# apache/tez

Measured on AMD Instinct MI355X. Metric: shuffled+sorted KV bytes/sec, higher is better.
Workload: dtype u8; 1 GPU; C2: 1e8 rec x (16B unique key + 64B val), 64 partitions, BytesWritable/TezBytesComparator, ordered shuffle; records=100000000, key_bytes=16, partitions=64, parallelism=single

## Files before the change

### tez_amd/csrc/tezsort.hip

```cpp
#include <hip/hip_runtime.h>
#include <cstdint>
#include <cstdio>
#include <cstdlib>
#include <cstring>
#include <string>
#include <vector>
#include <mutex>
#include <algorithm>
#include <sys/stat.h>
#include <sys/types.h>

#include "tezsort.h"

#define WAVE 64
#define BLOCK 256
#define WPB (BLOCK / WAVE)
#define RADIX 256
#define TILE_ROUNDS 12
#define TILE (TILE_ROUNDS * BLOCK)

static thread_local char g_err[1024];
extern "C" const char* tzs_last_error(void) { return g_err; }

#define FAIL(code, ...)                                        \
  do {                                                         \
    snprintf(g_err, sizeof(g_err), __VA_ARGS__);               \
    return (code);                                             \
  } while (0)

#define HIP_CHECK(x)                                                        \
  do {                                                                      \
    hipError_t _e = (x);                                                    \
    if (_e != hipSuccess)                                                   \
      FAIL(-70, "%s:%d HIP error %d (%s) in %s", __FILE__, __LINE__, (int)_e, \
           hipGetErrorString(_e), #x);                                      \
  } while (0)

static uint32_t h_crc_table[256];
static bool h_crc_init_done = false;
static void h_crc_init() {
  if (h_crc_init_done) return;
  for (uint32_t n = 0; n < 256; n++) {
    uint32_t c = n;
    for (int k = 0; k < 8; k++) c = (c & 1) ? (0xEDB88320u ^ (c >> 1)) : (c >> 1);
    h_crc_table[n] = c;
  }
  h_crc_init_done = true;
}
static uint32_t h_crc32(uint32_t crc, const uint8_t* p, size_t n) {
  h_crc_init();
  crc ^= 0xFFFFFFFFu;
  for (size_t i = 0; i < n; i++) crc = h_crc_table[(crc ^ p[i]) & 0xFF] ^ (crc >> 8);
  return crc ^ 0xFFFFFFFFu;
}

static uint32_t gf2_times(const uint32_t* m, uint32_t v) {
  uint32_t s = 0;
  for (int i = 0; v; i++, v >>= 1)
    if (v & 1) s ^= m[i];
  return s;
}
static void gf2_square(uint32_t* sq, const uint32_t* m) {
  for (int i = 0; i < 32; i++) sq[i] = gf2_times(m, m[i]);
}
#define CRC_MATS 40
static uint32_t h_crc_shift_mat[CRC_MATS][32];
static bool h_mats_done = false;
static void h_build_crc_mats() {
  if (h_mats_done) return;
  uint32_t odd[32], even[32];
  odd[0] = 0xEDB88320u;
  for (int i = 1; i < 32; i++) odd[i] = 1u << (i - 1);
  gf2_square(even, odd);
  gf2_square(odd, even);
  gf2_square(even, odd);
  memcpy(h_crc_shift_mat[0], even, sizeof(even));
  for (int k = 1; k < CRC_MATS; k++)
    gf2_square(h_crc_shift_mat[k], h_crc_shift_mat[k - 1]);
  h_mats_done = true;
}
static uint32_t h_crc_shift(uint32_t crc, uint64_t nbytes) {
  h_build_crc_mats();
  for (int k = 0; nbytes; k++, nbytes >>= 1)
    if (nbytes & 1) crc = gf2_times(h_crc_shift_mat[k], crc);
  return crc;
}
static uint32_t h_crc_combine(uint32_t c1, uint32_t c2, uint64_t len2) {
  return h_crc_shift(c1, len2) ^ c2;
}
extern "C" uint32_t tzs_test_crc_combine(uint32_t c1, uint32_t c2, uint64_t len2) {
  return h_crc_combine(c1, c2, len2);
}
extern "C" uint32_t tzs_test_crc32(uint32_t c, const void* p, uint64_t n) {
  return h_crc32(c, (const uint8_t*)p, n);
}

static int h_vint_size(int64_t i) {
  if (i >= -112 && i <= 127) return 1;
  if (i < 0) i = ~i;
  int n = 0;
  while (i != 0) { i = (int64_t)((uint64_t)i >> 8); n++; }
  return n + 1;
}

__device__ __forceinline__ int d_vint_size(int64_t i) {
  if (i >= -112 && i <= 127) return 1;
  uint64_t u = (i < 0) ? ~(uint64_t)i : (uint64_t)i;
  int n = 0;
  while (u != 0) { u >>= 8; n++; }
  return n + 1;
}
__device__ __forceinline__ int d_vint_write(uint8_t* b, int64_t i) {
  if (i >= -112 && i <= 127) { b[0] = (uint8_t)i; return 1; }
  int len = -112;
  if (i < 0) { i = ~i; len = -120; }
  int64_t tmp = i;
  while (tmp != 0) { tmp = (int64_t)((uint64_t)tmp >> 8); len--; }
  b[0] = (uint8_t)len;
  int n = (len < -120) ? -(len + 120) : -(len + 112);
  for (int idx = n; idx != 0; idx--)
    b[n - idx + 1] = (uint8_t)((uint64_t)i >> ((idx - 1) * 8));
  return n + 1;
}
__device__ __forceinline__ int d_vint_decoded_size(int8_t first) {
  if (first >= -112) return 1;
  if (first < -120) return -119 - first;
  return -111 - first;
}

__device__ __forceinline__ int32_t d_hash_bytes(const uint8_t* p, int32_t n) {
  if (n == 16) {
    uint64_t w0, w1;
    __builtin_memcpy(&w0, p, 8);
    __builtin_memcpy(&w1, p + 8, 8);
    int32_t A = 1, B = 0;
#pragma unroll
    for (int j = 0; j < 8; j++) {
      A = (int32_t)((uint32_t)A * 31u) + (int8_t)(uint8_t)(w0 >> (8 * j));
      B = (int32_t)((uint32_t)B * 31u) + (int8_t)(uint8_t)(w1 >> (8 * j));
    }
    uint32_t p8 = 1;
#pragma unroll
    for (int j = 0; j < 8; j++) p8 *= 31u;
    return (int32_t)((uint32_t)A * p8 + (uint32_t)B);
  }
  int32_t h = 1;
  int32_t i = 0;
  for (; i + 8 <= n; i += 8) {
    uint64_t w;
    __builtin_memcpy(&w, p + i, 8);
    for (int j = 0; j < 8; j++)
      h = (int32_t)((uint32_t)h * 31u) + (int8_t)(uint8_t)(w >> (8 * j));
  }
  for (; i < n; i++) h = (int32_t)((uint32_t)h * 31u) + (int8_t)p[i];
  return h;
}

struct SegDesc {
  const uint8_t* data;
  const uint64_t* off;
  const uint32_t* klen;
  uint32_t rec_u;
  uint32_t klen_u;
};
struct RecTable {
  const uint8_t* data0;
  const uint64_t* off0;
  const uint32_t* klen0;
  const SegDesc* segs;
  const uint32_t* base;
  uint32_t rec_u0, klen_u0;
  uint32_t n0;
  int32_t nspills;
  int32_t key_type;
};

__device__ __forceinline__ int rt_spill_of(const RecTable& rt, uint32_t g) {
  if (rt.nspills == 1 || g < rt.n0) return 0;
  uint32_t lo = 1, hi = (uint32_t)rt.nspills;
  while (lo + 1 < hi) {
    uint32_t mid = (lo + hi) >> 1;
    if (rt.base[mid] <= g) lo = mid; else hi = mid;
  }
  return (int)lo;
}
struct RecView {
  const uint8_t* key;
  uint32_t klen;
  const uint8_t* val;
  uint32_t vlen;
  const uint8_t* content;
  uint32_t clen;
};
__device__ __forceinline__ RecView rt_view(const RecTable& rt, uint32_t g) {
  const uint8_t* data;
  const uint64_t* off;
  const uint32_t* klen;
  uint32_t rec_u, klen_u, r;
  if (rt.nspills == 1 || g < rt.n0) {
    data = rt.data0; off = rt.off0; klen = rt.klen0;
    rec_u = rt.rec_u0; klen_u = rt.klen_u0; r = g;
  } else {
    int s = rt_spill_of(rt, g);
    SegDesc sd = rt.segs[s];
    data = sd.data; off = sd.off; klen = sd.klen;
    rec_u = sd.rec_u; klen_u = sd.klen_u; r = g - rt.base[s];
  }
  RecView v;
  if (rec_u) {
    v.key = data + (uint64_t)r * rec_u;
    v.klen = klen_u;
    v.val = v.key + v.klen;
    v.vlen = rec_u - v.klen;
  } else {
    uint64_t o = off[r];
    v.key = data + o;
    v.klen = klen[r];
    v.val = v.key + v.klen;
    v.vlen = (uint32_t)(off[r + 1] - o - v.klen);
  }
  if (rt.key_type == 1) {
    int n = d_vint_decoded_size((int8_t)v.key[0]);
    v.content = v.key + n;
    v.clen = v.klen - n;
  } else {
    v.content = v.key + 4;
    v.clen = v.klen - 4;
  }
  return v;
}

__global__ void k_shift_offsets(const uint64_t* src, uint64_t* dst, uint64_t shift,
                                int64_t n);
__global__ void k_max_u32(const uint32_t* a, uint32_t n, uint32_t* out);
__global__ void k_part_hist(const uint32_t* parts, uint32_t n, uint32_t* counts, int P);
__global__ void k_gather_part_meta(const uint64_t* pstart, const uint64_t* scan,
                                   const uint8_t* same, uint64_t total_body,
                                   uint32_t n, int P, uint64_t* out);
__global__ void k_check_uniform(const uint64_t* off, const uint32_t* klen, int64_t n,
                                uint64_t* mm );

__global__ void k_hash_partition(RecTable rt, int32_t P, int32_t* d_part, uint32_t n) {
  uint32_t stride = gridDim.x * blockDim.x;
  for (uint32_t i = blockIdx.x * blockDim.x + threadIdx.x; i < n; i += 2 * stride) {
    uint32_t j = i + stride;
    RecView v0 = rt_view(rt, i);
    int32_t h0 = d_hash_bytes(v0.content, (int32_t)v0.clen);
    if (j < n) {
      RecView v1 = rt_view(rt, j);
      int32_t h1 = d_hash_bytes(v1.content, (int32_t)v1.clen);
      d_part[j] = (h1 & 0x7fffffff) % P;
    }
    d_part[i] = (h0 & 0x7fffffff) % P;
  }
}

__device__ __forceinline__ uint64_t d_composite_one(
    const RecTable& rt, const int32_t* d_part, int32_t P, int pbits,
    int ref_pb, int ser_mode, uint64_t mask, uint32_t i) {
  RecView v = rt_view(rt, i);
  uint32_t part;
  if (d_part) part = (uint32_t)d_part[i];
  else part = (uint32_t)((d_hash_bytes(v.content, (int32_t)v.clen) & 0x7fffffff) % P);
  uint64_t key;
  if (ser_mode) {
    uint32_t proxy = ((v.clen > 0 ? (uint32_t)v.content[0] : 0u) << 16) |
                     ((v.clen > 1 ? (uint32_t)v.content[1] : 0u) << 8) |
                     (v.clen > 2 ? (uint32_t)v.content[2] : 0u);
    int pw = 24 - ref_pb;
    if (pw < 0) pw = 0;
    uint32_t proxy_t = pw ? (proxy >> (24 - pw)) : 0;
    uint64_t ser = 0;
    uint32_t m = v.klen < 8 ? v.klen : 8;
    for (uint32_t b = 0; b < m; b++) ser |= (uint64_t)v.key[b] << (56 - 8 * b);
    key = ((uint64_t)part << (64 - pbits))
          | ((uint64_t)proxy_t << (64 - pbits - pw))
          | (ser >> (pbits + pw));
  } else {
    uint64_t c = 0;
    uint32_t m = v.clen < 8 ? v.clen : 8;
    for (uint32_t b = 0; b < m; b++) c |= (uint64_t)v.content[b] << (56 - 8 * b);
    key = pbits ? (((uint64_t)part << (64 - pbits)) | (c >> pbits)) : c;
  }
  return key & mask;
}

__global__ void k_build_composite2(RecTable rt, const int32_t* d_part, int32_t P,
                                   int pbits, int ref_pb, int sort_bytes,
                                   int ser_mode, uint64_t* d_key, uint32_t* d_idx,
                                   uint32_t n) {
  uint64_t mask = (sort_bytes >= 8) ? ~0ull : ~0ull << (8 * (8 - sort_bytes));
  uint32_t stride = gridDim.x * blockDim.x;
  for (uint32_t i = blockIdx.x * blockDim.x + threadIdx.x; i < n; i += 4 * stride) {
    uint32_t i1 = i + stride, i2 = i + 2 * stride, i3 = i + 3 * stride;
    uint64_t k0 = d_composite_one(rt, d_part, P, pbits, ref_pb, ser_mode, mask, i);
    uint64_t k1 = (i1 < n) ? d_composite_one(rt, d_part, P, pbits, ref_pb,
                                             ser_mode, mask, i1) : 0;
    uint64_t k2 = (i2 < n) ? d_composite_one(rt, d_part, P, pbits, ref_pb,
                                             ser_mode, mask, i2) : 0;
    uint64_t k3 = (i3 < n) ? d_composite_one(rt, d_part, P, pbits, ref_pb,
                                             ser_mode, mask, i3) : 0;
    d_key[i] = k0;
    d_idx[i] = i;
    if (i1 < n) { d_key[i1] = k1; d_idx[i1] = i1; }
    if (i2 < n) { d_key[i2] = k2; d_idx[i2] = i2; }
    if (i3 < n) { d_key[i3] = k3; d_idx[i3] = i3; }
  }
}

__global__ void k_build_composite(RecTable rt, const int32_t* d_part, int32_t P,
                                  int pbits, int ref_pb, int sort_bytes, int ser_mode,
                                  uint64_t* d_key, uint32_t* d_idx, uint32_t n) {
  uint64_t mask = (sort_bytes >= 8) ? ~0ull : ~0ull << (8 * (8 - sort_bytes));
  for (uint32_t i = blockIdx.x * blockDim.x + threadIdx.x; i < n;
       i += gridDim.x * blockDim.x) {
    RecView v = rt_view(rt, i);
    uint32_t part;
    if (d_part) part = (uint32_t)d_part[i];
    else part = (uint32_t)((d_hash_bytes(v.content, (int32_t)v.clen) & 0x7fffffff) % P);
    uint64_t key;
    if (ser_mode) {
      uint32_t proxy = ((v.clen > 0 ? (uint32_t)v.content[0] : 0u) << 16) |
                       ((v.clen > 1 ? (uint32_t)v.content[1] : 0u) << 8) |
                       (v.clen > 2 ? (uint32_t)v.content[2] : 0u);
      int pw = 24 - ref_pb;
      if (pw < 0) pw = 0;
      uint32_t proxy_t = pw ? (proxy >> (24 - pw)) : 0;
      uint64_t ser = 0;
      uint32_t m = v.klen < 8 ? v.klen : 8;
      for (uint32_t b = 0; b < m; b++) ser |= (uint64_t)v.key[b] << (56 - 8 * b);
      key = ((uint64_t)part << (64 - pbits))
            | ((uint64_t)proxy_t << (64 - pbits - pw))
            | (ser >> (pbits + pw));
    } else {
      uint64_t c = 0;
      uint32_t m = v.clen < 8 ? v.clen : 8;
      for (uint32_t b = 0; b < m; b++) c |= (uint64_t)v.content[b] << (56 - 8 * b);
      key = pbits ? (((uint64_t)part << (64 - pbits)) | (c >> pbits)) : c;
    }
    d_key[i] = key & mask;
    d_idx[i] = i;
  }
}

template <typename KeyT, int BLK = BLOCK>
__global__ void k_radix_hist(const KeyT* keys, uint32_t n, int byte_idx,
                             uint32_t* counts ) {
  constexpr uint32_t OT = (uint32_t)TILE_ROUNDS * BLK;
  __shared__ uint32_t h[RADIX];
  for (int i = threadIdx.x; i < RADIX; i += blockDim.x) h[i] = 0;
  __syncthreads();
  uint32_t start = blockIdx.x * OT;
  uint32_t end = min(start + OT, n);
  for (uint32_t i = start + threadIdx.x; i < end; i += blockDim.x) {
    uint32_t d = (uint32_t)(keys[i] >> (8 * byte_idx)) & 0xFF;
    atomicAdd(&h[d], 1u);
  }
  __syncthreads();
  for (int i = threadIdx.x; i < RADIX; i += blockDim.x)
    counts[blockIdx.x * RADIX + i] = h[i];
}

__global__ void k_radix_scan_blocks(const uint32_t* counts, uint32_t nblocks,
                                    uint32_t* offsets, uint32_t* totals) {
  int d = blockIdx.x;
  __shared__ uint32_t lds[BLOCK];
  uint32_t running = 0;
  for (uint32_t b0 = 0; b0 < nblocks; b0 += blockDim.x) {
    uint32_t b = b0 + threadIdx.x;
    uint32_t v = (b < nblocks) ? counts[b * RADIX + d] : 0;
    lds[threadIdx.x] = v;
    __syncthreads();
    for (int s = 1; s < BLOCK; s <<= 1) {
      uint32_t t = (threadIdx.x >= (uint32_t)s) ? lds[threadIdx.x - s] : 0;
      __syncthreads();
      lds[threadIdx.x] += t;
      __syncthreads();
    }
    if (b < nblocks) offsets[b * RADIX + d] = running + lds[threadIdx.x] - v;
    uint32_t chunk_total = lds[BLOCK - 1];
    running += chunk_total;
    __syncthreads();
  }
  if (threadIdx.x == 0) totals[d] = running;
}

__global__ void k_radix_scan_digits(uint32_t* totals, uint32_t* bases) {
  __shared__ uint32_t lds[RADIX];
  int t = threadIdx.x;
  lds[t] = totals[t];
  __syncthreads();
  for (int s = 1; s < RADIX; s <<= 1) {
    uint32_t v = (t >= s) ? lds[t - s] : 0;
    __syncthreads();
    lds[t] += v;
    __syncthreads();
  }
  bases[t] = lds[t] - totals[t];
}

template <typename KeyT, bool HAS_A1, bool HAS_B64 = false, int BLK = BLOCK>
__global__ __launch_bounds__(BLK) void k_radix_scatter(
    const KeyT* keys_in, KeyT* keys_out,
    const uint32_t* a0_in, uint32_t* a0_out,
    const uint32_t* a1_in, uint32_t* a1_out,
    const uint64_t* b64_in, uint64_t* b64_out,
    uint32_t n, int byte_idx,
    const uint32_t* offsets, const uint32_t* bases) {
  constexpr uint32_t OT = (uint32_t)TILE_ROUNDS * BLK;
  constexpr int OWPB = BLK / WAVE;
  constexpr int RW = OWPB * TILE_ROUNDS;
  constexpr size_t CNT_BYTES = (size_t)RW * RADIX * 2;
  constexpr size_t KEY_BYTES = (size_t)OT * sizeof(KeyT);
  constexpr size_t UNION_BYTES = CNT_BYTES > KEY_BYTES ? CNT_BYTES : KEY_BYTES;
  __shared__ __attribute__((aligned(16))) uint8_t u_raw[UNION_BYTES];
  __shared__ uint32_t ls_a0[OT];
  __shared__ uint32_t ls_a1[HAS_A1 ? OT : 1];
  __shared__ uint64_t ls_b64[HAS_B64 ? OT : 1];
  __shared__ uint32_t tileoff[RADIX];
  uint16_t* cnt = (uint16_t*)u_raw;
  KeyT* ls_key = (KeyT*)u_raw;
  for (uint32_t i = threadIdx.x; i < (uint32_t)RW * RADIX / 2; i += blockDim.x)
    ((uint32_t*)cnt)[i] = 0;
  __syncthreads();
  uint32_t start = blockIdx.x * OT;
  uint32_t end = min(start + OT, n);
  uint32_t count = (start < n) ? (end - start) : 0;
  const int lane = threadIdx.x & (WAVE - 1);
  const int wv = threadIdx.x / WAVE;
  const uint64_t lt_mask = (lane == 0) ? 0ull : (~0ull >> (64 - lane));
  KeyT my_key[TILE_ROUNDS];
  uint32_t my_a0[TILE_ROUNDS];
  uint32_t my_a1v[HAS_A1 ? TILE_ROUNDS : 1];
  uint64_t my_b64[HAS_B64 ? TILE_ROUNDS : 1];
  uint16_t my_rank[TILE_ROUNDS];
  uint16_t my_dig[TILE_ROUNDS];
  #pragma unroll
  for (int r = 0; r < TILE_ROUNDS; r++) {
    uint32_t i = start + (uint32_t)r * BLK + threadIdx.x;
    bool active = i < end;
    my_key[r] = active ? keys_in[i] : (KeyT)0;
    my_a0[r] = active ? a0_in[i] : 0;
    if (HAS_A1) my_a1v[r] = active ? a1_in[i] : 0;
    if (HAS_B64) my_b64[r] = active ? b64_in[i] : 0;
  }
  for (int r = 0; r < TILE_ROUNDS; r++) {
    uint32_t i = start + (uint32_t)r * BLK + threadIdx.x;
    bool active = i < end;
    uint32_t d = active ? ((uint32_t)(my_key[r] >> (8 * byte_idx)) & 0xFF) : 0u;
    uint64_t m = ~0ull;
    for (int b = 0; b < 8; b++) {
      uint64_t bb = __ballot((d >> b) & 1);
      m &= ((d >> b) & 1) ? bb : ~bb;
    }
    uint64_t act = __ballot(active);
    m &= act;
    uint32_t lane_rank = (uint32_t)__popcll(m & lt_mask);
    if (active && lane_rank == 0)
      cnt[(r * OWPB + wv) * RADIX + d] = (uint16_t)__popcll(m);
    my_rank[r] = (uint16_t)lane_rank;
    my_dig[r] = (uint16_t)d;
  }
  __syncthreads();
  if (threadIdx.x < RADIX) {
    uint32_t d = threadIdx.x;
    uint32_t running = 0;
    for (int rw = 0; rw < RW; rw++) {
      uint32_t t = cnt[rw * RADIX + d];
      cnt[rw * RADIX + d] = (uint16_t)running;
      running += t;
    }
    tileoff[d] = running;
  }
  __syncthreads();
  if (wv == 0) {
    uint32_t v0 = tileoff[4 * lane], v1 = tileoff[4 * lane + 1],
             v2 = tileoff[4 * lane + 2], v3 = tileoff[4 * lane + 3];
    uint32_t sum = v0 + v1 + v2 + v3;
    uint32_t inc = sum;
    for (int s2 = 1; s2 < WAVE; s2 <<= 1) {
      uint32_t t = __shfl_up(inc, s2);
      if (lane >= s2) inc += t;
    }
    uint32_t base0 = inc - sum;
    tileoff[4 * lane] = base0;
    tileoff[4 * lane + 1] = base0 + v0;
    tileoff[4 * lane + 2] = base0 + v0 + v1;
    tileoff[4 * lane + 3] = base0 + v0 + v1 + v2;
  }
  __syncthreads();
  uint16_t my_slot[TILE_ROUNDS];
  for (int r = 0; r < TILE_ROUNDS; r++) {
    uint32_t d = my_dig[r];
    my_slot[r] = (uint16_t)(tileoff[d] + cnt[(r * OWPB + wv) * RADIX + d] +
                            my_rank[r]);
  }
  __syncthreads();
  for (int r = 0; r < TILE_ROUNDS; r++) {
    uint32_t i = start + (uint32_t)r * BLK + threadIdx.x;
    if (i < end) {
      uint32_t slot = my_slot[r];
      ls_key[slot] = my_key[r];
      ls_a0[slot] = my_a0[r];
      if (HAS_A1) ls_a1[slot] = my_a1v[r];
      if (HAS_B64) ls_b64[slot] = my_b64[r];
    }
  }
  __syncthreads();
  for (uint32_t j = threadIdx.x; j < count; j += blockDim.x) {
    KeyT k = ls_key[j];
    uint32_t d = (uint32_t)(k >> (8 * byte_idx)) & 0xFF;
    uint32_t pos = offsets[blockIdx.x * RADIX + d] + bases[d] + (j - tileoff[d]);
    keys_out[pos] = k;
    a0_out[pos] = ls_a0[j];
    if (HAS_A1) a1_out[pos] = ls_a1[j];
    if (HAS_B64) b64_out[pos] = ls_b64[j];
  }
}

#define OS_AGG (1u << 30)
#define OS_INC (2u << 30)
#define OS_CNT_MASK ((1u << 30) - 1)
typedef unsigned int __attribute__((address_space(1))) os_gu32;

template <typename KeyT>
__global__ void k_global_hist_all(const KeyT* keys, uint32_t n, int first_byte,
                                  int npasses, uint32_t* counts ) {
  extern __shared__ uint32_t lh[];
  for (int i = threadIdx.x; i < npasses * RADIX; i += blockDim.x) lh[i] = 0;
  __syncthreads();
  for (uint32_t i = blockIdx.x * blockDim.x + threadIdx.x; i < n;
       i += gridDim.x * blockDim.x) {
    KeyT k = keys[i];
    for (int p = 0; p < npasses; p++)
      atomicAdd(&lh[p * RADIX + ((uint32_t)(k >> (8 * (first_byte + p))) & 0xFF)], 1u);
  }
  __syncthreads();
  for (int i = threadIdx.x; i < npasses * RADIX; i += blockDim.x)
    if (lh[i]) atomicAdd(&counts[i], lh[i]);
}

__global__ void k_os_bases(const uint32_t* counts, uint32_t* bases) {
  __shared__ uint32_t tot[RADIX];
  int p = blockIdx.x;
  int d = threadIdx.x;
  tot[d] = counts[p * RADIX + d];
  __syncthreads();
  if (d == 0) {
    uint32_t run = 0;
    for (int i = 0; i < RADIX; i++) {
      uint32_t t = tot[i];
      tot[i] = run;
      run += t;
    }
  }
  __syncthreads();
  bases[p * RADIX + d] = tot[d];
}

template <typename KeyT, bool HAS_A1, bool HAS_B64 = false, int BLK = BLOCK>
__global__ __launch_bounds__(BLK) void k_onesweep_pass(
    const KeyT* keys_in, KeyT* keys_out,
    const uint32_t* a0_in, uint32_t* a0_out,
    const uint32_t* a1_in, uint32_t* a1_out,
    const uint64_t* b64_in, uint64_t* b64_out,
    uint32_t n, int byte_idx,
    const uint32_t* bases ,
    uint32_t* status , uint32_t* ticket, uint32_t* error) {
  constexpr uint32_t OT = (uint32_t)TILE_ROUNDS * BLK;
  constexpr int OWPB = BLK / WAVE;
  constexpr int RW = OWPB * TILE_ROUNDS;
  constexpr size_t CNT_BYTES = (size_t)RW * RADIX * 2;
  constexpr size_t KEY_BYTES = (size_t)OT * sizeof(KeyT);
  constexpr size_t UNION_BYTES = CNT_BYTES > KEY_BYTES ? CNT_BYTES : KEY_BYTES;
  __shared__ __attribute__((aligned(16))) uint8_t u_raw[UNION_BYTES];
  __shared__ uint32_t ls_a0[OT];
  __shared__ uint32_t ls_a1[HAS_A1 ? OT : 1];
  __shared__ uint64_t ls_b64[HAS_B64 ? OT : 1];
  __shared__ uint32_t tileoff[RADIX];
  __shared__ uint32_t excl[RADIX];
  __shared__ uint32_t s_tile;
  uint16_t* cnt = (uint16_t*)u_raw;
  KeyT* ls_key = (KeyT*)u_raw;
  if (threadIdx.x == 0) s_tile = atomicAdd(ticket, 1u);
  for (uint32_t i = threadIdx.x; i < (uint32_t)RW * RADIX / 2; i += blockDim.x)
    ((uint32_t*)cnt)[i] = 0;
  __syncthreads();
  const uint32_t tile = s_tile;
  const uint32_t start = tile * OT;
  const uint32_t end = min(start + OT, n);
  const uint32_t count = (start < n) ? (end - start) : 0;
  const int lane = threadIdx.x & (WAVE - 1);
  const int wv = threadIdx.x / WAVE;
  const uint64_t lt_mask = (lane == 0) ? 0ull : (~0ull >> (64 - lane));
  KeyT my_key[TILE_ROUNDS];
  uint32_t my_a0[TILE_ROUNDS];
  uint32_t my_a1v[HAS_A1 ? TILE_ROUNDS : 1];
  uint64_t my_b64[HAS_B64 ? TILE_ROUNDS : 1];
  uint16_t my_rank[TILE_ROUNDS];
  uint16_t my_dig[TILE_ROUNDS];
  #pragma unroll
  for (int r = 0; r < TILE_ROUNDS; r++) {
    uint32_t i = start + (uint32_t)r * BLK + threadIdx.x;
    bool active = i < end;
    my_key[r] = active ? keys_in[i] : (KeyT)0;
    my_a0[r] = active ? a0_in[i] : 0;
    if (HAS_A1) my_a1v[r] = active ? a1_in[i] : 0;
    if (HAS_B64) my_b64[r] = active ? b64_in[i] : 0;
  }
// ... 2230 lines not shown
  uint32_t cur_rec_u = 0;
  uint32_t cur_klen_u = 0;
  bool cur_first_batch = true;
  bool have_explicit_parts = false;
  bool combined_parts_valid = false;
  DBuf combine_data, combine_off, combine_klen;
  uint32_t combine_n = 0;
  bool combine_applied = false;
  std::vector<uint8_t> host_data;
  std::vector<uint64_t> host_off;
  std::vector<uint32_t> host_klen;
  std::vector<int32_t> host_part;
  std::vector<SpillData*> spills;
  DBuf final_ifile;
  int64_t final_len = 0;
  std::vector<tzs_index_record> final_index;
  bool flushed = false;
  tzs_counters ctr = {};
  tzs_times times = {};
  DBuf skey, sidx, eq, same, sizes, scan, parts_sorted;
  DBuf skey_lo;
  DBuf comp_ifile;
  int64_t comp_len = 0;
  std::vector<tzs_index_record> comp_index;
  std::vector<uint64_t> final_rec_ranges;
  HostRT final_hrt;
  RecTable final_rt = {};
  uint32_t final_n = 0;
  DBuf col_data, col_off, col_klen;
};

extern "C" void tzs_conf_default(tzs_conf* c, int32_t num_partitions) {
  memset(c, 0, sizeof(*c));
  c->num_partitions = num_partitions;
  c->key_type = TZS_KEY_BYTES;
  c->value_type = TZS_KEY_BYTES;
  c->comparator = TZS_CMP_TEZBYTES;
  c->rle = -1;
  c->send_empty_partition_details = 1;
  c->io_sort_factor = 100;
  c->final_merge_enabled = 1;
  c->sort_buffer_bytes = 100ll << 20;
  c->device = -1;
  c->world_size = 1;
  c->rank = 0;
  c->combiner = 0;
  c->min_spills_for_combine = 3;
  c->discard_spill_streams = 0;
}

extern "C" int tzs_sorter_create(const tzs_conf* conf, tzs_sorter** out) {
  if (!conf || conf->num_partitions <= 0) FAIL(-22, "bad conf");
  if (ensure_device_constants()) return -70;
  tzs_sorter* s = new tzs_sorter();
  s->conf = *conf;
  s->pbits = pbits_for(conf->num_partitions);
  *out = s;
  return 0;
}

extern "C" int tzs_sorter_write(tzs_sorter* s, const void* key, int32_t klen,
                                const void* val, int32_t vlen, int32_t partition) {
  if (s->host_off.empty()) s->host_off.push_back(0);
  const uint8_t* k = (const uint8_t*)key;
  const uint8_t* v = (const uint8_t*)val;
  s->host_data.insert(s->host_data.end(), k, k + klen);
  s->host_data.insert(s->host_data.end(), v, v + vlen);
  s->host_off.push_back(s->host_data.size());
  s->host_klen.push_back((uint32_t)klen);
  s->host_part.push_back(partition);
  if ((int64_t)s->host_data.size() + 16ll * (int64_t)s->host_klen.size()
      > s->conf.sort_buffer_bytes)
    return tzs_sorter_spill(s);
  return 0;
}

static int absorb_host_staging(tzs_sorter* s) {
  if (s->host_klen.empty()) return 0;
  int64_t n = (int64_t)s->host_klen.size();
  static_assert(sizeof(uint64_t) == 8, "");
  DBuf dd, doff, dkl, dpart;
  if (dd.alloc(s->host_data.size() ? s->host_data.size() : 1)) return -12;
  if (doff.alloc(sizeof(uint64_t) * (n + 1))) return -12;
  if (dkl.alloc(sizeof(uint32_t) * n)) return -12;
  if (dpart.alloc(sizeof(int32_t) * n)) return -12;
  HIP_CHECK(hipMemcpy(dd.p, s->host_data.data(), s->host_data.size(), hipMemcpyHostToDevice));
  HIP_CHECK(hipMemcpy(doff.p, s->host_off.data(), sizeof(uint64_t) * (n + 1), hipMemcpyHostToDevice));
  HIP_CHECK(hipMemcpy(dkl.p, s->host_klen.data(), sizeof(uint32_t) * n, hipMemcpyHostToDevice));
  bool have_parts = true;
  for (auto p : s->host_part) if (p < 0) { have_parts = false; break; }
  HIP_CHECK(hipMemcpy(dpart.p, s->host_part.data(), sizeof(int32_t) * n, hipMemcpyHostToDevice));
  int rc = tzs_sorter_write_batch_device(s, dd.p, (const uint64_t*)doff.p,
                                         (const uint32_t*)dkl.p,
                                         have_parts ? (const int32_t*)dpart.p : nullptr, n);
  dd.release(); doff.release(); dkl.release(); dpart.release();
  s->host_data.clear(); s->host_off.clear(); s->host_klen.clear(); s->host_part.clear();
  return rc;
}

#include <chrono>
extern "C" int tzs_sorter_write_batch_device(tzs_sorter* s, const void* d_data,
                                             const uint64_t* d_off, const uint32_t* d_klen,
                                             const int32_t* d_part, int64_t n) {
  auto t0 = std::chrono::steady_clock::now();
  if (n == 0) return 0;
  if (n > 4000000000ll) FAIL(-22, "batch too large (u32 record ids)");
  uint64_t nbytes = 0, first = 0;
  HIP_CHECK(hipMemcpy(&first, d_off, 8, hipMemcpyDeviceToHost));
  HIP_CHECK(hipMemcpy(&nbytes, d_off + n, 8, hipMemcpyDeviceToHost));
  nbytes -= first;
  if (first != 0) FAIL(-22, "d_off must start at 0");

  uint64_t old_bytes = s->cur_bytes;
  int64_t old_n = s->cur_n;
  DBuf nd, noff, nkl, npart;
  if (nd.alloc(old_bytes + nbytes ? old_bytes + nbytes : 1)) return -12;
  if (noff.alloc(sizeof(uint64_t) * (old_n + n + 1))) return -12;
  if (nkl.alloc(sizeof(uint32_t) * (old_n + n))) return -12;
  if (npart.alloc(sizeof(int32_t) * (old_n + n))) return -12;
  if (old_n) {
    HIP_CHECK(hipMemcpyAsync(nd.p, s->cur_data.p, old_bytes, hipMemcpyDeviceToDevice));
    HIP_CHECK(hipMemcpyAsync(noff.p, s->cur_off.p, sizeof(uint64_t) * old_n, hipMemcpyDeviceToDevice));
    HIP_CHECK(hipMemcpyAsync(nkl.p, s->cur_klen.p, sizeof(uint32_t) * old_n, hipMemcpyDeviceToDevice));
    HIP_CHECK(hipMemcpyAsync(npart.p, s->cur_part.p, sizeof(int32_t) * old_n, hipMemcpyDeviceToDevice));
  }
  HIP_CHECK(hipMemcpyAsync((uint8_t*)nd.p + old_bytes, d_data, nbytes, hipMemcpyDeviceToDevice));
  HIP_CHECK(hipMemcpyAsync((uint32_t*)nkl.p + old_n, d_klen, sizeof(uint32_t) * n, hipMemcpyDeviceToDevice));
  hipLaunchKernelGGL(k_shift_offsets, dim3(grid1d(n + 1)), dim3(BLOCK), 0, 0,
                     d_off, (uint64_t*)noff.p + old_n, old_bytes, n + 1);
  std::swap(s->cur_data, nd); nd.release();
  std::swap(s->cur_off, noff); noff.release();
  std::swap(s->cur_klen, nkl); nkl.release();
  if (d_part) {
    HIP_CHECK(hipMemcpyAsync((int32_t*)npart.p + old_n, d_part, sizeof(int32_t) * n,
                             hipMemcpyDeviceToDevice));
    s->have_explicit_parts = true;
  } else if (s->have_explicit_parts) {
    FAIL(-22, "cannot mix explicit and computed partitions in one sorter");
  }
  std::swap(s->cur_part, npart); npart.release();
  {
    static thread_local DBuf mm;
    if (mm.alloc(32)) return -12;
    uint64_t init[4] = {~0ull, 0, ~0ull, 0};
    HIP_CHECK(hipMemcpyAsync(mm.p, init, 32, hipMemcpyHostToDevice));
    hipLaunchKernelGGL(k_check_uniform, dim3(grid1d(n)), dim3(BLOCK), 0, 0,
                       d_off, d_klen, n, (uint64_t*)mm.p);
    uint64_t res[4];
    HIP_CHECK(hipMemcpy(res, mm.p, 32, hipMemcpyDeviceToHost));
    bool uni = (res[0] == res[1]) && (res[2] == res[3]) && res[0] <= 0xFFFFFFFFull;
    if (getenv("TZS_NO_UNIFORM")) uni = false;
    if (s->cur_first_batch) {
      s->cur_rec_u = uni ? (uint32_t)res[0] : 0;
      s->cur_klen_u = uni ? (uint32_t)res[2] : 0;
      s->cur_first_batch = false;
    } else if (!uni || s->cur_rec_u != (uint32_t)res[0] ||
               s->cur_klen_u != (uint32_t)res[2]) {
      s->cur_rec_u = 0;
      s->cur_klen_u = 0;
    }
  }
  s->cur_n = old_n + n;
  s->cur_bytes = old_bytes + nbytes;
  s->ctr.output_records += n;
  s->ctr.output_bytes += (int64_t)nbytes;
  HIP_CHECK(hipDeviceSynchronize());
  s->times.absorb_ns += std::chrono::duration_cast<std::chrono::nanoseconds>(
      std::chrono::steady_clock::now() - t0).count();
  return 0;
}

extern "C" int tzs_sorter_write_batch_device_adopt(tzs_sorter* s, void* d_data,
                                                   uint64_t* d_off, uint32_t* d_klen,
                                                   int32_t* d_part, int64_t n) {
  auto t0 = std::chrono::steady_clock::now();
  if (n == 0) return 0;
  if (n > 4000000000ll) FAIL(-22, "batch too large (u32 record ids)");
  if (s->cur_n != 0 || !s->host_klen.empty())
    FAIL(-22, "adopt requires an empty current buffer (first batch of spill)");
  std::unique_lock<std::mutex> reg_lk(pool_mu());
  auto& reg = pool_registry();
  auto id = reg.find(d_data), io = reg.find(d_off), ik = reg.find(d_klen);
  auto ip = d_part ? reg.find(d_part) : reg.end();
  if (id == reg.end() || io == reg.end() || ik == reg.end() ||
      (d_part && ip == reg.end()))
    FAIL(-22, "adopt requires buffers allocated by tzs_malloc_device/tzs_generate");
  size_t cls_d = id->second, cls_o = io->second, cls_k = ik->second;
  size_t cls_p = d_part ? ip->second : 0;
  reg_lk.unlock();
  uint64_t nbytes = 0;
  bool hinted = false;
  {
    std::lock_guard<std::mutex> lk(pool_mu());
    auto hh = uniform_hints().find(d_off);
    if (hh != uniform_hints().end() && !getenv("TZS_NO_UNIFORM")) {
      s->cur_rec_u = hh->second.rec_u;
      s->cur_klen_u = hh->second.klen_u;
      nbytes = hh->second.nbytes;
      s->cur_first_batch = false;
      uniform_hints().erase(hh);
      hinted = true;
    }
  }
  if (!hinted) {
    uint64_t first = 0;
    HIP_CHECK(hipMemcpy(&first, d_off, 8, hipMemcpyDeviceToHost));
    HIP_CHECK(hipMemcpy(&nbytes, d_off + n, 8, hipMemcpyDeviceToHost));
    if (first != 0) FAIL(-22, "d_off must start at 0");
    static thread_local DBuf mm;
    if (mm.alloc(32)) return -12;
    uint64_t init[4] = {~0ull, 0, ~0ull, 0};
    HIP_CHECK(hipMemcpyAsync(mm.p, init, 32, hipMemcpyHostToDevice));
    hipLaunchKernelGGL(k_check_uniform, dim3(grid1d(n)), dim3(BLOCK), 0, 0,
                       d_off, d_klen, n, (uint64_t*)mm.p);
    uint64_t res[4];
    HIP_CHECK(hipMemcpy(res, mm.p, 32, hipMemcpyDeviceToHost));
    bool uni = (res[0] == res[1]) && (res[2] == res[3]) && res[0] <= 0xFFFFFFFFull;
    if (getenv("TZS_NO_UNIFORM")) uni = false;
    s->cur_rec_u = uni ? (uint32_t)res[0] : 0;
    s->cur_klen_u = uni ? (uint32_t)res[2] : 0;
    s->cur_first_batch = false;
  }
  {
    std::lock_guard<std::mutex> lk(pool_mu());
    reg.erase(d_data);
    reg.erase(d_off);
    reg.erase(d_klen);
    if (d_part) reg.erase(d_part);
  }
  s->cur_data.release(); s->cur_data.p = d_data; s->cur_data.sz = cls_d;
  s->cur_off.release();  s->cur_off.p = d_off;   s->cur_off.sz = cls_o;
  s->cur_klen.release(); s->cur_klen.p = d_klen; s->cur_klen.sz = cls_k;
  if (d_part) {
    s->cur_part.release(); s->cur_part.p = d_part; s->cur_part.sz = cls_p;
    s->have_explicit_parts = true;
  } else {
    if (s->cur_part.alloc(sizeof(int32_t) * n)) return -12;
    s->have_explicit_parts = false;
  }
  s->cur_n = n;
  s->cur_bytes = nbytes;
  s->ctr.output_records += n;
  s->ctr.output_bytes += (int64_t)nbytes;
  HIP_CHECK(hipDeviceSynchronize());
  s->times.absorb_ns += std::chrono::duration_cast<std::chrono::nanoseconds>(
      std::chrono::steady_clock::now() - t0).count();
  return 0;
}

__global__ void k_shift_offsets(const uint64_t* src, uint64_t* dst, uint64_t shift,
                                int64_t n) {
  for (int64_t i = blockIdx.x * blockDim.x + threadIdx.x; i < n;
       i += (int64_t)gridDim.x * blockDim.x)
    dst[i] = src[i] + shift;
}

struct SortParams {
  int ser_mode;
  int SB;
  int ref_pb;
  int proxy_w;
};
static SortParams derive_sort_params(tzs_sorter* s,
                                     const std::vector<SegDesc>& hsegs,
                                     uint32_t n) {
  SortParams sp;
  int P = s->conf.num_partitions;
  int pbits = s->pbits;
  sp.ser_mode = (s->conf.comparator == TZS_CMP_TEZBYTES) ? 1 : 0;
  if (sp.ser_mode) {
    bool uniform_klen = !hsegs.empty();
    uint32_t k0 = hsegs.empty() ? 0 : hsegs[0].klen_u;
    for (auto& sd : hsegs)
      if (sd.klen_u == 0 || sd.klen_u != k0) { uniform_klen = false; break; }
    if (uniform_klen && k0 != 0) sp.ser_mode = 0;
  }
  sp.ref_pb = 1;
  for (int v2 = P; v2; v2 >>= 1) sp.ref_pb++;
  sp.proxy_w = 24 - sp.ref_pb;
  if (sp.proxy_w < 0) sp.proxy_w = 0;
  int needed_bits = pbits + 6;
  for (uint64_t v = n; v; v >>= 1) needed_bits++;
  int SB = (needed_bits + 7) / 8;
  if (SB < 2) SB = 2;
  if (sp.ser_mode) {
    int minsb = (pbits + sp.proxy_w + 7) / 8;
    if (SB < minsb) SB = minsb;
  }
  if (s->conf.comparator == TZS_CMP_TEXT) {
    SB = 8;
  }
  if (SB > 8) SB = 8;
  sp.SB = SB;
  return sp;
}

static int refine_and_emit(tzs_sorter* s, std::vector<SegDesc> hsegs,
                           std::vector<uint32_t> hbase,
                           RecTable rt, uint32_t n, int SB, int ser_mode,
                           const uint8_t* h_spill_rle, int nspills_rle,
                           SpillData* outsp, bool apply_combine,
                           SpillData* retain, const uint64_t* d_lo);

static int sort_and_emit(tzs_sorter* s, HostRT& hrt, uint32_t n,
                         const int32_t* d_part_unsorted,
                         const uint8_t* h_spill_rle, int nspills_rle,
                         SpillData* outsp, bool apply_combine = false,
                         SpillData* retain = nullptr) {
  tzs_times& T = s->times;
  g_scatter_ns = 0; g_scatter_launches = 0; g_scatter_elems = 0;
  hipEvent_t ev[4];
  for (auto& e : ev) (void)hipEventCreate(&e);
  (void)hipEventRecord(ev[0]);

  RecTable rt = hrt.rt;
  int P = s->conf.num_partitions;
  int pbits = s->pbits;
  SortParams prm = derive_sort_params(s, hrt.segs, n);
  int ser_mode = prm.ser_mode, SB = prm.SB;
  if (s->skey.alloc(sizeof(uint64_t) * n)) return -12;
  if (s->sidx.alloc(sizeof(uint32_t) * n)) return -12;
  uint64_t* d_key = (uint64_t*)s->skey.p;
  uint32_t* d_idx = (uint32_t*)s->sidx.p;
  hipLaunchKernelGGL(k_build_composite2, dim3(grid1d(n)), dim3(BLOCK), 0, 0, rt,
                     d_part_unsorted, P, pbits, prm.ref_pb, SB, ser_mode, d_key,
                     d_idx, n);
  (void)hipEventRecord(ev[1]);

  int rc = radix_sort<uint64_t>(d_key, d_idx, nullptr, n, 8, 8 - SB,
                                &s->skey, &s->sidx, nullptr);
  if (rc) return rc;
  (void)hipEventRecord(ev[2]);
  (void)hipEventSynchronize(ev[2]);
  float ms = 0;
  (void)hipEventElapsedTime(&ms, ev[0], ev[1]); T.composite_ns += (int64_t)(ms * 1e6);
  (void)hipEventElapsedTime(&ms, ev[1], ev[2]); T.sort_ns += (int64_t)(ms * 1e6);
  (void)hipEventElapsedTime(&ms, ev[0], ev[2]); T.total_ns += (int64_t)(ms * 1e6);
  for (auto& e : ev) (void)hipEventDestroy(e);
  return refine_and_emit(s, hrt.segs, hrt.base, rt, n, SB, ser_mode,
                         h_spill_rle, nspills_rle, outsp, apply_combine,
                         retain, nullptr);
}

static int refine_and_emit(tzs_sorter* s, std::vector<SegDesc> hsegs,
                           std::vector<uint32_t> hbase,
                           RecTable rt, uint32_t n, int SB, int ser_mode,
                           const uint8_t* h_spill_rle, int nspills_rle,
                           SpillData* outsp, bool apply_combine,
                           SpillData* retain, const uint64_t* d_lo) {
  tzs_times& T = s->times;
  hipEvent_t ev[10];
  for (auto& e : ev) (void)hipEventCreate(&e);
  int P = s->conf.num_partitions;
  int pbits = s->pbits;
  int ref_pb = 1;
  for (int v2 = P; v2; v2 >>= 1) ref_pb++;
  int proxy_w = 24 - ref_pb;
  if (proxy_w < 0) proxy_w = 0;
  uint64_t* d_key = (uint64_t*)s->skey.p;
  uint32_t* d_idx = (uint32_t*)s->sidx.p;
  int rc = 0;
  (void)hipEventRecord(ev[2]);

  if (s->eq.alloc(n)) return -12;
  if (s->parts_sorted.alloc(sizeof(uint32_t) * n)) return -12;
  uint8_t* d_eq = (uint8_t*)s->eq.p;
  if (d_lo)
    hipLaunchKernelGGL(k_eq_init2, dim3(grid1d(n)), dim3(BLOCK), 0, 0, d_key,
                       d_lo, d_eq, pbits, (uint32_t*)s->parts_sorted.p, n);
  else
    hipLaunchKernelGGL(k_eq_init, dim3(grid1d(n)), dim3(BLOCK), 0, 0, d_key, d_eq,
                       pbits, (uint32_t*)s->parts_sorted.p, n);
  int c0 = ser_mode ? (8 * SB - pbits - proxy_w) / 8 : (8 * SB - pbits) / 8;
  if (c0 < 0) c0 = 0;
  int c0_eff = d_lo ? c0 + 8 : c0;
  uint32_t max_klen = 0;
  {
    bool need_dev = false;
    for (size_t sp = 0; sp < hsegs.size(); sp++) {
      if (hsegs[sp].klen_u) {
        if (hsegs[sp].klen_u > max_klen) max_klen = hsegs[sp].klen_u;
      } else {
        need_dev = true;
      }
    }
    if (need_dev) {
      static thread_local DBuf dmax;
      if (dmax.alloc(4)) return -12;
      HIP_CHECK(hipMemsetAsync(dmax.p, 0, 4));
      for (size_t sp = 0; sp < hsegs.size(); sp++) {
        if (hsegs[sp].klen_u) continue;
        uint32_t cnt = hbase[sp + 1] - hbase[sp];
        if (!cnt) continue;
        hipLaunchKernelGGL(k_max_u32, dim3(grid1d(cnt)), dim3(BLOCK), 0, 0,
                           hsegs[sp].klen, cnt, (uint32_t*)dmax.p);
      }
      uint32_t dm = 0;
      HIP_CHECK(hipMemcpy(&dm, dmax.p, 4, hipMemcpyDeviceToHost));
      if (dm > max_klen) max_klen = dm;
    }
  }
  int max_clen = (int)max_klen;
  static thread_local DBuf eqcnt;
  static thread_local DBuf lkey, seg, pos, slotpos;
  static thread_local DBuf lk0;
  if (eqcnt.alloc(4)) return -12;

  bool will_combine = apply_combine && s->conf.combiner == 1;
  bool lk0_retain_ready = false;
  int level = 1;
  const int max_levels = (max_clen > c0_eff) ? (max_clen - c0_eff + 7) / 8 : 0;
  uint32_t neq = 0;
  {
    HIP_CHECK(hipMemsetAsync(eqcnt.p, 0, 4));
    hipLaunchKernelGGL(k_count_nonzero_u8, dim3(grid1d(n)), dim3(BLOCK), 0, 0, d_eq, n,
                       (uint32_t*)eqcnt.p);
    HIP_CHECK(hipMemcpy(&neq, eqcnt.p, 4, hipMemcpyDeviceToHost));
  }
  for (int li = 0; li <= max_levels; li++) {
    if (neq == 0) break;
    int use_len = (li == max_levels);
    uint64_t mcap64 = 2ull * neq;
    uint32_t mcap = (uint32_t)(mcap64 < n ? mcap64 : n);
    if (lkey.alloc(sizeof(uint64_t) * mcap)) return -12;
    if (seg.alloc(sizeof(uint32_t) * mcap)) return -12;
    if (pos.alloc(sizeof(uint32_t) * mcap)) return -12;
    int lb0 = c0_eff + 8 * li;
    uint64_t ptotal = 0;
    {
      const uint64_t* lk0p = nullptr;
      if (3ull * neq >= n && n <= 300000000u && !lk0_retain_ready) {
        if (lk0.alloc(8ull * n)) return -12;
        hipLaunchKernelGGL(k_build_lkeys, dim3(grid1d(n)), dim3(BLOCK), 0, 0, rt,
                           lb0, use_len, ser_mode, (uint64_t*)lk0.p, n);
        lk0p = (const uint64_t*)lk0.p;
      }
      static thread_local DBuf rc_st, rc_tick;
      uint32_t nb_rc = nblocks_for(n, SCAN_TILE);
      if (rc_st.alloc(8ull * nb_rc)) return -12;
      if (rc_tick.alloc(32)) return -12;
      HIP_CHECK(hipMemsetAsync(rc_st.p, 0, 8ull * nb_rc));
      HIP_CHECK(hipMemsetAsync(rc_tick.p, 0, 32));
      hipLaunchKernelGGL(k_refine_compact_lb, dim3(nb_rc), dim3(BLOCK), 0, 0, rt,
                         d_idx, d_eq, n, lb0, use_len, ser_mode, lk0p,
                         (uint64_t*)lkey.p, (uint32_t*)seg.p, (uint32_t*)pos.p,
                         (uint64_t*)rc_st.p, (uint32_t*)rc_tick.p,
                         (uint32_t*)rc_tick.p + 1, (uint64_t*)rc_tick.p + 2);
      uint64_t hh[3] = {0, 0, 0};
      HIP_CHECK(hipMemcpy(hh, rc_tick.p, 24, hipMemcpyDeviceToHost));
      if ((uint32_t)(hh[0] >> 32)) FAIL(-70, "refine compact lookback timeout");
      ptotal = hh[2];
      if (li == 0 && !use_len && lk0p && retain && !will_combine)
        lk0_retain_ready = true;
      else if (!lk0_retain_ready)
        lk0.release();
    }
    uint64_t nruns = ptotal & 0xFFFFFFFFu;
    uint32_t m = (uint32_t)(ptotal >> 32);
    if (m == 0) break;
    if (slotpos.alloc(sizeof(uint32_t) * m)) return -12;
    HIP_CHECK(hipMemcpyAsync(slotpos.p, pos.p, sizeof(uint32_t) * m,
                             hipMemcpyDeviceToDevice));
    int segbytes = 1;
    while ((nruns >> (8 * segbytes)) != 0 && segbytes < 4) segbytes++;
    rc = radix_sort<uint64_t>((uint64_t*)lkey.p, (uint32_t*)seg.p, (uint32_t*)pos.p, m, 8);
    if (rc) return rc;
    rc = radix_sort<uint32_t>((uint32_t*)seg.p, (uint32_t*)pos.p, nullptr, m, segbytes,
                              0, nullptr, nullptr, nullptr, (uint64_t*)lkey.p, &lkey);
    if (rc) return rc;
    static thread_local DBuf idx_tmp;
    if (idx_tmp.alloc(sizeof(uint32_t) * m)) return -12;
    hipLaunchKernelGGL(k_refine_gather, dim3(grid1d(m)), dim3(BLOCK), 0, 0,
                       (const uint32_t*)pos.p, d_idx, (uint32_t*)idx_tmp.p, m);
    hipLaunchKernelGGL(k_refine_scatter, dim3(grid1d(m)), dim3(BLOCK), 0, 0,
                       (const uint32_t*)slotpos.p, (const uint32_t*)idx_tmp.p,
                       d_idx, m);
    HIP_CHECK(hipMemsetAsync(eqcnt.p, 0, 4));
    hipLaunchKernelGGL(k_eq_update, dim3(grid1d(m)), dim3(BLOCK), 0, 0,
                       (const uint64_t*)lkey.p, (const uint32_t*)seg.p,
                       (const uint32_t*)slotpos.p, d_eq, m, (uint32_t*)eqcnt.p);
    HIP_CHECK(hipMemcpy(&neq, eqcnt.p, 4, hipMemcpyDeviceToHost));
    level++;
  }
  (void)hipEventRecord(ev[3]);
  lkey.release(); seg.release(); pos.release(); slotpos.release();
  radix_release_temps();

  if (retain && !will_combine) {
    std::swap(retain->skey, s->skey);
    if (retain->sidxb.alloc(4ull * n)) return -12;
    HIP_CHECK(hipMemcpyAsync(retain->sidxb.p, s->sidx.p, 4ull * n,
                             hipMemcpyDeviceToDevice));
    if (retain->skey2.alloc(8ull * n)) return -12;
    {
      if (!lk0_retain_ready) {
        if (lk0.alloc(8ull * n)) return -12;
        hipLaunchKernelGGL(k_build_lkeys, dim3(grid1d(n)), dim3(BLOCK), 0, 0, rt,
                           c0, 0, ser_mode, (uint64_t*)lk0.p, n);
      }
      hipLaunchKernelGGL(k_gather_merge_hi, dim3(grid1d(n)), dim3(BLOCK), 0, 0,
                         (const uint64_t*)lk0.p, (const uint32_t*)s->sidx.p,
                         (uint64_t*)retain->skey2.p, 0ull, n);
      lk0.release();
    }
    retain->lo_c0 = c0;
    retain->sort_sb = SB;
    retain->sort_ser_mode = ser_mode;
    retain->sorted_valid = 1;
  }

  uint32_t neq_final = neq;
  int writer_rle;
  if (s->conf.rle >= 0) {
    writer_rle = s->conf.rle;
  } else if (nspills_rle > 1) {
    if (s->same.alloc(n)) return -12;
    {
      static thread_local DBuf d_sprle0, cnt0;
      if (d_sprle0.alloc(nspills_rle)) return -12;
      if (cnt0.alloc(4)) return -12;
      HIP_CHECK(hipMemcpyAsync(d_sprle0.p, h_spill_rle, nspills_rle,
                               hipMemcpyHostToDevice));
      hipLaunchKernelGGL(k_writer_same, dim3(grid1d(n)), dim3(BLOCK), 0, 0, rt,
                         d_idx, d_eq, 0, (const uint8_t*)d_sprle0.p,
                         (uint8_t*)s->same.p, n);
      HIP_CHECK(hipMemsetAsync(cnt0.p, 0, 4));
      hipLaunchKernelGGL(k_count_nonzero_u8, dim3(grid1d(n)), dim3(BLOCK), 0, 0,
                         (const uint8_t*)s->same.p, n, (uint32_t*)cnt0.p);
      uint32_t ev = 0;
      HIP_CHECK(hipMemcpy(&ev, cnt0.p, 4, hipMemcpyDeviceToHost));
      writer_rle = ((uint64_t)ev * 10 > n) ? 1 : 0;
    }
  } else {
    writer_rle = ((uint64_t)neq_final * 10 > n) ? 1 : 0;
  }

  s->combine_applied = false;
  if (apply_combine && s->conf.combiner == 1) {
    static thread_local DBuf rs, rs_scan, pos2, lens2, off2, parts2, idx2;
    if (rs.alloc(8ull * n) || rs_scan.alloc(8ull * n)) return -12;
    hipLaunchKernelGGL(k_combine_mark, dim3(grid1d(n)), dim3(BLOCK), 0, 0, d_eq,
                       (uint64_t*)rs.p, n);
    uint64_t M64 = 0;
    if (scan_u64((uint64_t*)rs.p, (uint64_t*)rs_scan.p, n, &M64)) return -12;
    uint32_t M = (uint32_t)M64;
    if (pos2.alloc(4ull * M) || lens2.alloc(8ull * M) || off2.alloc(8ull * (M + 1)))
      return -12;
    hipLaunchKernelGGL(k_combine_pos, dim3(grid1d(n)), dim3(BLOCK), 0, 0, d_eq,
                       (const uint64_t*)rs_scan.p, (uint32_t*)pos2.p,
                       (uint64_t*)lens2.p, rt, d_idx, n);
    uint64_t bytes2 = 0;
    if (scan_u64((uint64_t*)lens2.p, (uint64_t*)off2.p, M, &bytes2)) return -12;
    HIP_CHECK(hipMemcpy((uint64_t*)off2.p + M, &bytes2, 8, hipMemcpyHostToDevice));
    if (s->combine_data.alloc(bytes2 ? bytes2 : 1)) return -12;
    if (s->combine_klen.alloc(4ull * M)) return -12;
    if (parts2.alloc(4ull * M) || idx2.alloc(4ull * M)) return -12;
    hipLaunchKernelGGL(k_combine_fold, dim3(grid_waves(M)), dim3(BLOCK), 0, 0, rt,
                       d_idx, (const uint32_t*)pos2.p, (const uint64_t*)off2.p,
                       (const uint32_t*)s->parts_sorted.p, (uint8_t*)s->combine_data.p,
                       (uint32_t*)s->combine_klen.p, (uint32_t*)parts2.p, M, n);
    std::swap(s->combine_off, off2);
    RecTable rt2 = {};
    rt2.nspills = 1;
    rt2.data0 = (const uint8_t*)s->combine_data.p;
    rt2.off0 = (const uint64_t*)s->combine_off.p;
    rt2.klen0 = (const uint32_t*)s->combine_klen.p;
    rt2.n0 = M;
    rt2.key_type = rt.key_type;
    rt = rt2;
    n = M;
    SegDesc csd;
    csd.data = rt2.data0; csd.off = rt2.off0; csd.klen = rt2.klen0;
    csd.rec_u = 0; csd.klen_u = 0;
    hsegs.assign(1, csd);
    hbase.assign(2, 0);
    hbase[1] = M;
    hipLaunchKernelGGL(k_iota, dim3(grid1d(n)), dim3(BLOCK), 0, 0,
                       (uint32_t*)idx2.p, n);
    std::swap(s->sidx, idx2);
    d_idx = (uint32_t*)s->sidx.p;
    if (s->eq.alloc(n)) return -12;
    d_eq = (uint8_t*)s->eq.p;
    HIP_CHECK(hipMemsetAsync(d_eq, 0, n));
    std::swap(s->parts_sorted, parts2);
    writer_rle = 0;
    s->combined_parts_valid = true;
    s->combine_applied = true;
    s->combine_n = M;
    if (retain) {
      s->skey.release();
      if (retain->skey.alloc(8ull * n)) return -12;
      if (retain->sidxb.alloc(4ull * n)) return -12;
      hipLaunchKernelGGL(k_build_composite, dim3(grid1d(n)), dim3(BLOCK), 0, 0,
                         rt, (const int32_t*)s->parts_sorted.p, P, pbits,
                         ref_pb, SB, ser_mode, (uint64_t*)retain->skey.p,
                         (uint32_t*)retain->sidxb.p, n);
      if (retain->skey2.alloc(8ull * n)) return -12;
      hipLaunchKernelGGL(k_build_lkeys, dim3(grid1d(n)), dim3(BLOCK), 0, 0, rt,
                         c0, 0, ser_mode, (uint64_t*)retain->skey2.p, n);
      retain->lo_c0 = c0;
      retain->sort_sb = SB;
      retain->sort_ser_mode = ser_mode;
      retain->sorted_valid = 1;
    }
  } else {
    s->combined_parts_valid = false;
  }
  if (s->same.alloc(n)) return -12;
  static thread_local DBuf d_sprle;
  if (d_sprle.alloc(nspills_rle ? nspills_rle : 1)) return -12;
  if (nspills_rle)
    HIP_CHECK(hipMemcpy(d_sprle.p, h_spill_rle, nspills_rle, hipMemcpyHostToDevice));
  hipLaunchKernelGGL(k_writer_same, dim3(grid1d(n)), dim3(BLOCK), 0, 0, rt, d_idx, d_eq,
                     writer_rle, (const uint8_t*)d_sprle.p, (uint8_t*)s->same.p, n);

  uint32_t uni_rec = 0, uni_klen = 0;
  {
    bool uni = !hsegs.empty() && !s->combine_applied;
    for (size_t sp2 = 0; sp2 < hsegs.size() && uni; sp2++) {
      if (!hsegs[sp2].rec_u || !hsegs[sp2].klen_u) uni = false;
      else if (sp2 == 0) { uni_rec = hsegs[0].rec_u; uni_klen = hsegs[0].klen_u; }
      else if (uni_rec != hsegs[sp2].rec_u || uni_klen != hsegs[sp2].klen_u)
        uni = false;
    }
    if (!uni) uni_rec = 0;
  }
  bool no_same = (writer_rle == 0) &&
      (neq_final == 0 || (nspills_rle == 1 && h_spill_rle && !h_spill_rle[0]));
  uint32_t uh_len = 0;
// ... 1163 lines not shown
```

Before: 341.2 billion bytes/s.

## Add wave-cooperative coalesced composite-key builder for uniform fixed-size records

Adds a specialized composite-key kernel for single-spill, fixed-size records. Each wave loads a contiguous run of 64 records with coalesced 16-byte vector loads, stages them in LDS, and then each lane hashes and extracts its own key prefix from LDS. This replaces the scattered per-record byte reads in the generic builder. It is gated by record-size, alignment and an env override, and adds per-NV template instantiations and extra LDS use.

```diff
diff --git a/tez_amd/csrc/tezsort.hip b/tez_amd/csrc/tezsort.hip
--- a/tez_amd/csrc/tezsort.hip
+++ b/tez_amd/csrc/tezsort.hip
@@ -305,6 +305,68 @@
     if (i1 < n) { d_key[i1] = k1; d_idx[i1] = i1; }
     if (i2 < n) { d_key[i2] = k2; d_idx[i2] = i2; }
     if (i3 < n) { d_key[i3] = k3; d_idx[i3] = i3; }
+  }
+}
+
+template <int NV >
+__global__ __launch_bounds__(BLOCK) void k_build_composite_stream(
+    const uint8_t* __restrict__ data0, const int32_t* __restrict__ d_part,
+    int32_t P, int pbits, int sort_bytes, uint32_t rec_u,
+    uint32_t clen ,
+    uint64_t* __restrict__ d_key, uint32_t* __restrict__ d_idx, uint32_t n) {
+  extern __shared__ uint4 cs_lds[];
+  const uint32_t W = rec_u >> 2;
+  const uint32_t nvec = 16 * W;
+  const uint32_t lane = threadIdx.x & (WAVE - 1);
+  const uint32_t wib = threadIdx.x / WAVE;
+  uint4* L4 = cs_lds + wib * (NV * WAVE);
+  const uint32_t* mine = (const uint32_t*)L4 + lane * W + 1;
+  const uint64_t mask = (sort_bytes >= 8) ? ~0ull : ~0ull << (8 * (8 - sort_bytes));
+  const uint32_t cbytes = d_part ? (clen < 8 ? clen : 8) : clen;
+  const uint32_t nw = (cbytes + 3) >> 2;
+  const uint64_t ngroups = ((uint64_t)n + WAVE - 1) / WAVE;
+  const uint32_t nwaves = gridDim.x * (BLOCK / WAVE);
+  for (uint64_t g = blockIdx.x * (BLOCK / WAVE) + wib; g < ngroups; g += nwaves) {
+    const uint64_t base = g * WAVE;
+    const uint64_t i = base + lane;
+    int32_t h = 1;
+    uint64_t c = 0;
+    if (base + WAVE <= n) {
+      const uint4* src = (const uint4*)(data0 + base * rec_u);
+      uint4 v[NV];
+#pragma unroll
+      for (int j = 0; j < NV; j++) {
+        uint32_t t = j * WAVE + lane;
+        v[j] = src[(j < NV - 1 || t < nvec) ? t : nvec - 1];
+      }
+#pragma unroll
+      for (int j = 0; j < NV; j++) L4[j * WAVE + lane] = v[j];
+      __builtin_amdgcn_wave_barrier();
+      for (uint32_t j = 0; j < nw; j++) {
+        uint32_t x = mine[j];
+        uint32_t nb = cbytes - 4 * j < 4 ? cbytes - 4 * j : 4;
+        if (!d_part)
+          for (uint32_t b = 0; b < nb; b++)
+            h = (int32_t)((uint32_t)h * 31u) + (int8_t)(uint8_t)(x >> (8 * b));
+        if (j < 2) {
+          if (nb < 4) x &= (1u << (8 * nb)) - 1u;
+          c |= (uint64_t)__builtin_bswap32(x) << (32 * (1 - j));
+        }
+      }
+      __builtin_amdgcn_wave_barrier();
+    } else if (i < n) {
+      const uint8_t* ct = data0 + i * rec_u + 4;
+      if (!d_part) h = d_hash_bytes(ct, (int32_t)clen);
+      uint32_t m = clen < 8 ? clen : 8;
+      for (uint32_t b = 0; b < m; b++) c |= (uint64_t)ct[b] << (56 - 8 * b);
+    }
+    if (i < n) {
+      uint32_t part = d_part ? (uint32_t)d_part[i]
+                             : (uint32_t)((h & 0x7fffffff) % P);
+      uint64_t key = pbits ? (((uint64_t)part << (64 - pbits)) | (c >> pbits)) : c;
+      d_key[i] = key & mask;
+      d_idx[i] = (uint32_t)i;
+    }
   }
 }
 
@@ -3141,6 +3203,14 @@
                            SpillData* outsp, bool apply_combine,
                            SpillData* retain, const uint64_t* d_lo);
 
+static bool stream_uniform_gate(const RecTable& rt) {
+  const char* e = getenv("TZS_STREAM_UNIFORM");
+  if (e && e[0] == '0') return false;
+  return rt.nspills == 1 && rt.key_type == 0 && rt.rec_u0 != 0 &&
+         rt.klen_u0 >= 4 && rt.klen_u0 <= rt.rec_u0 && rt.rec_u0 % 4 == 0 &&
+         rt.rec_u0 <= 128 && ((uintptr_t)rt.data0 & 15) == 0;
+}
+
 static int sort_and_emit(tzs_sorter* s, HostRT& hrt, uint32_t n,
                          const int32_t* d_part_unsorted,
                          const uint8_t* h_spill_rle, int nspills_rle,
@@ -3161,9 +3231,23 @@
   if (s->sidx.alloc(sizeof(uint32_t) * n)) return -12;
   uint64_t* d_key = (uint64_t*)s->skey.p;
   uint32_t* d_idx = (uint32_t*)s->sidx.p;
-  hipLaunchKernelGGL(k_build_composite2, dim3(grid1d(n)), dim3(BLOCK), 0, 0, rt,
-                     d_part_unsorted, P, pbits, prm.ref_pb, SB, ser_mode, d_key,
-                     d_idx, n);
+  if (ser_mode == 0 && stream_uniform_gate(rt)) {
+#define TZS_CS_LAUNCH(NV)                                                     \
+  case NV:                                                                    \
+    hipLaunchKernelGGL((k_build_composite_stream<NV>), dim3(grid1d(n)),       \
+                       dim3(BLOCK), (BLOCK / WAVE) * NV * WAVE * 16, 0,       \
+                       rt.data0, d_part_unsorted, P, pbits, SB, rt.rec_u0,    \
+                       rt.klen_u0 - 4, d_key, d_idx, n);                      \
+    break;
+    switch ((rt.rec_u0 + 15) / 16) {
+      TZS_CS_LAUNCH(1) TZS_CS_LAUNCH(2) TZS_CS_LAUNCH(3) TZS_CS_LAUNCH(4)
+      TZS_CS_LAUNCH(5) TZS_CS_LAUNCH(6) TZS_CS_LAUNCH(7) TZS_CS_LAUNCH(8)
+    }
+#undef TZS_CS_LAUNCH
+  } else
+    hipLaunchKernelGGL(k_build_composite2, dim3(grid1d(n)), dim3(BLOCK), 0, 0, rt,
+                       d_part_unsorted, P, pbits, prm.ref_pb, SB, ser_mode, d_key,
+                       d_idx, n);
   (void)hipEventRecord(ev[1]);
 
   int rc = radix_sort<uint64_t>(d_key, d_idx, nullptr, n, 8, 8 - SB,
```

Measured after the change: 378.4 billion bytes/s, median of 6. 10.9% higher.
